# QI2lab/ray_trace_pb

Hardware: AMD Instinct MI355X
Metric: ray-surface intersections/sec at 1/2/4/8 MI355X; achieved HBM GB/s vs peak (higher is better)
Workload: dtype f64

## Files before the change

ray_trace_pb_amd/csrc/rtpb_core.hip:

```cpp
#include "rtpb_internal.h"

namespace rtpbi {

thread_local std::string g_last_error;

int fail(int code, const std::string& msg) {
    g_last_error = msg;
    return code;
}

PinnedStaging& pinned_staging() {
    thread_local PinnedStaging sg;
    return sg;
}

template <typename T>
void blob_layout(rtpb_plan& p) {
    p.off_mats = align256(p.surf.size() * sizeof(DevSurface<T>));
    p.off_table = p.off_mats + align256(p.mats.size() * sizeof(DevMaterial<T>));
    p.off_itab = p.off_table + align256(std::max<size_t>(p.table.size(), 2) * sizeof(T));
    p.blob_bytes = p.off_itab + align256(std::max<size_t>(p.itab.size(), 2) * sizeof(T));
}

DevMaterial<double> device_material(const rtpb_plan& p, size_t k) {
    const rtpb_material& m = p.mats[k];
    DevMaterial<double> d{};
    d.kind = m.kind;
    bool zero = m.kind == RTPB_SELLMEIER;
    for (int j = 0; j < 6; ++j) {
        d.c[j] = m.c[j];
        zero = zero && m.c[j] == 0.0;
    }
    if (zero) d.kind = VACUUM;
    d.table_off = p.table_off[k];
    d.table_len = m.kind == RTPB_TABLE ? m.table_len : 0;
    return d;
}

void build_indexed(rtpb_plan& p) {
    if (p.table.empty() || (p.feat & 2)) return;
    const size_t M = p.mats.size();
    int first = -1;
    for (size_t k = 0; k < M; ++k)
        if (p.mats[k].kind == RTPB_TABLE) { first = static_cast<int>(k); break; }
    if (first < 0) return;
    const int K = p.mats[first].table_len;
    const size_t S = p.surf.size();
    if (K <= 0 || static_cast<size_t>(K) * (M + 1 + S) > static_cast<size_t>(kLdsIndexedDoubles)) return;
    const double* keys0 = p.table.data() + 2 * static_cast<size_t>(p.table_off[first]);
    for (int j = 0; j < K; ++j) {
        const double kj = keys0[2 * j];
        if (kj != kj && j != K - 1) return;
        if (j > 0 && kj == kj && !(keys0[2 * (j - 1)] < kj)) return;
    }
    for (size_t k = 0; k < M; ++k) {
        if (p.mats[k].kind != RTPB_TABLE) continue;
        if (p.mats[k].table_len != K) return;
        const double* kk = p.table.data() + 2 * static_cast<size_t>(p.table_off[k]);
        for (int j = 0; j < K; ++j) {
            const double a = kk[2 * j], b = keys0[2 * j];
            if (a != a ? b == b : std::memcmp(&a, &b, sizeof(double)) != 0) return;
        }
    }
    std::vector<double> it(static_cast<size_t>(K) * (M + 1 + S));
    for (int j = 0; j < K; ++j) it[j] = keys0[2 * j];
    for (size_t k = 0; k < M; ++k) {
        const double* kk = p.table.data() + 2 * static_cast<size_t>(p.table_off[k]);
        const DevMaterial<double> d = device_material(p, k);
        for (int j = 0; j < K; ++j)
            it[K * (k + 1) + j] = p.mats[k].kind == RTPB_TABLE ? kk[2 * j + 1]
                                                               : material_n<double, false, false>(d, keys0[2 * j], static_cast<const double*>(nullptr));
    }
    for (size_t s = 0; s < S; ++s)
        for (int j = 0; j < K; ++j) it[K * (M + 1 + s) + j] = it[K * (s + 1) + j] / it[K * (s + 2) + j];
    p.itab.swap(it);
    p.nkeys = K;
    p.feat = (p.feat & ~(4 | 8)) | 16;
}

template <typename T>
std::vector<unsigned char> build_blob(const rtpb_plan& p) {
    const size_t S = p.surf.size(), M = p.mats.size(), off_mats = p.off_mats, off_table = p.off_table;
    std::vector<unsigned char> blob(p.blob_bytes, 0);
    auto* ds = reinterpret_cast<DevSurface<T>*>(blob.data());
    for (size_t k = 0; k < S; ++k) {
        DevSurface<double> d = lower_surface(p.surf[k]);
        lower_surface_media(d, device_material(p, k), device_material(p, k + 1));
        DevSurface<T>& o = ds[k];
        o.kind = d.kind;
        for (int j = 0; j < 3; ++j) {
            o.c[j] = T(d.c[j]);
            o.nrm[j] = T(d.nrm[j]);
            o.ax[j] = T(d.ax[j]);
        }
        o.R = T(d.R); o.R2 = T(d.R2); o.absR = T(d.absR); o.ap = T(d.ap); o.f = T(d.f); o.sin_a = T(d.sin_a);
        o.tol = T(d.tol); o.ap_sq = T(d.ap_sq); o.shell_lo = T(d.shell_lo); o.shell_hi = T(d.shell_hi);
        o.rR = T(d.rR); o.rf = T(d.rf); o.rcp_ok = d.rcp_ok;
        for (int j = 0; j < 3; ++j) o.nf[j] = T(d.nf[j]);
        o.nr = T(d.nr); o.rn2 = T(d.rn2);
        for (int j = 0; j < 3; ++j) {
            o.lF[j] = T(d.lF[j]);
            o.lB[j] = T(d.lB[j]);
        }
        o.ln1f = T(d.ln1f); o.lph = T(d.lph);
    }
    auto* dm = reinterpret_cast<DevMaterial<T>*>(blob.data() + off_mats);
    for (size_t k = 0; k < M; ++k) dm[k] = device_material(p, k);
    auto* tb = reinterpret_cast<T*>(blob.data() + off_table);
    for (size_t k = 0; k < p.table.size(); ++k) tb[k] = T(p.table[k]);
    auto* it = reinterpret_cast<T*>(blob.data() + p.off_itab);
    for (size_t k = 0; k < p.itab.size(); ++k) it[k] = T(p.itab[k]);
    return blob;
}

int plan_device_blob(rtpb_plan* p, int dev, void** out) {
    std::lock_guard<std::mutex> lk(p->mu);
    if (!p->blob[dev]) {
        std::vector<unsigned char> host = build_blob<double>(*p);
        DeviceGuard g(dev);
        void* d = nullptr;
        HIP_TRY(hipMalloc(&d, host.size()));
        hipError_t e = hipMemcpy(d, host.data(), host.size(), hipMemcpyHostToDevice);
        if (e != hipSuccess) {
            (void)hipFree(d);
            return fail(RTPB_E_HIP, std::string("hipMemcpy(plan): ") + hipGetErrorString(e));
        }
        p->blob[dev] = d;
    }
    *out = p->blob[dev];
    return RTPB_OK;
}

int check_device(int dev) {
    int n = 0;
    if (hipGetDeviceCount(&n) != hipSuccess || n <= 0) return fail(RTPB_E_NODEV, "no GPU device visible");
    if (dev < 0 || dev >= n || dev >= kMaxDevices)
        return fail(RTPB_E_NODEV, "device index " + std::to_string(dev) + " out of range");
    return RTPB_OK;
}

}

using namespace rtpbi;

extern "C" {

int rtpb_abi_version(void) { return RTPB_ABI_VERSION; }

const char* rtpb_last_error(void) { return g_last_error.c_str(); }

int rtpb_device_count(void) {
    int n = 0;
    if (hipGetDeviceCount(&n) != hipSuccess) return 0;
    return n;
}

int rtpb_plan_create(const rtpb_surface* surfaces, int32_t nsurf, const rtpb_material* materials, int32_t nmat,
                     int32_t dtype, rtpb_plan** plan_out) {
    if (!plan_out) return fail(RTPB_E_INVALID, "plan_out is NULL");
    *plan_out = nullptr;
    if (nsurf < 0 || (nsurf > 0 && !surfaces)) return fail(RTPB_E_INVALID, "bad surfaces array");
    if (nsurf > RTPB_MAX_SURFACES)
        return fail(RTPB_E_LIMIT, "more than RTPB_MAX_SURFACES (" + std::to_string(RTPB_MAX_SURFACES) + ") surfaces");
    if (nmat != nsurf + 1 || !materials)
        return fail(RTPB_E_INVALID, "length of materials should be len(surfaces) + 1");
    if (dtype != RTPB_F64 && dtype != RTPB_F32) return fail(RTPB_E_INVALID, "dtype must be RTPB_F64 or RTPB_F32");
    auto* p = new (std::nothrow) rtpb_plan();
    if (!p) return fail(RTPB_E_INVALID, "out of host memory");
    p->dtype = dtype;
    p->nsurf = nsurf;
    for (int k = 0; k < nsurf; ++k) {
        if (surfaces[k].kind < RTPB_FLAT || surfaces[k].kind > RTPB_PERFECT_LENS) {
            delete p;
            return fail(RTPB_E_INVALID, "surface " + std::to_string(k) + ": unknown kind");
        }
        p->surf.push_back(surfaces[k]);
        if (surfaces[k].kind == RTPB_PERFECT_LENS) p->feat |= 1;
    }
    for (int k = 0; k < nmat; ++k) {
        rtpb_material m = materials[k];
        if (m.kind < RTPB_CONSTANT || m.kind > RTPB_TABLE) {
            delete p;
            return fail(RTPB_E_INVALID, "material " + std::to_string(k) + ": unknown kind");
        }
        p->table_off.push_back(static_cast<int32_t>(p->table.size() / 2));
        if (m.kind == RTPB_POLY6) p->feat |= 3;
        if (m.kind == RTPB_TABLE) {
            if (m.table_len <= 0 || !m.table) {
                delete p;
                return fail(RTPB_E_INVALID, "material " + std::to_string(k) + ": empty table");
            }
            if (p->table.size() / 2 + m.table_len > RTPB_MAX_TABLE) {
                delete p;
                return fail(RTPB_E_LIMIT, "more than RTPB_MAX_TABLE wavelength table entries");
            }
            p->table.insert(p->table.end(), m.table, m.table + 2 * m.table_len);
            sort_table(p->table.data() + p->table.size() - 2 * m.table_len, m.table_len);
        }
        m.table = nullptr;
        p->mats.push_back(m);
    }
    if (!p->table.empty()) p->feat |= (p->table.size() / 2 <= static_cast<size_t>(kLdsTablePairs)) ? 4 : 8;
    if (g_indexed_materials.load()) build_indexed(*p);
    if (p->feat == 1) {
        bool lens_flat = true;
        for (const rtpb_surface& s : p->surf) {
            const DevSurface<double> d = lower_surface(s);
            lens_flat = lens_flat && (d.kind == FLAT || d.kind == PERFECT_LENS) &&
                        surface_geo(d.kind, d.rcp_ok) != kGeoGeneral;
        }
        if (lens_flat) p->feat |= 32;
    }
    blob_layout<double>(*p);
    *plan_out = p;
    return RTPB_OK;
}

int rtpb_plan_destroy(rtpb_plan* plan) {
    if (!plan) return RTPB_OK;
    for (int d = 0; d < kMaxDevices; ++d) {
        if (plan->blob[d]) {
            DeviceGuard g(d);
            (void)hipFree(plan->blob[d]);
        }
    }
    delete plan;
    return RTPB_OK;
}

}
```

ray_trace_pb_amd/csrc/rtpb_internal.h:

```cpp
#pragma once

#include <hip/hip_runtime.h>

#include <atomic>
#include <cmath>
#include <cstdio>
#include <cstring>
#include <mutex>
#include <string>
#include <thread>
#include <vector>

#include "rtpb.h"
#include "rtpb_math.h"

namespace rtpbi {

using namespace rtpb;

constexpr int kBlock = 256;
constexpr int kTraceBlock = 64;
constexpr int kMaxDevices = 64;

extern thread_local std::string g_last_error;
int fail(int code, const std::string& msg);

#define HIP_TRY(expr)                                                                          \
    do {                                                                                       \
        hipError_t e_ = (expr);                                                                \
        if (e_ != hipSuccess)                                                                  \
            return fail(RTPB_E_HIP, std::string(#expr ": ") + hipGetErrorString(e_));          \
    } while (0)

struct DeviceGuard {
    int prev = -1;
    explicit DeviceGuard(int dev) {
        if (hipGetDevice(&prev) != hipSuccess) prev = -1;
        if (prev != dev) (void)hipSetDevice(dev);
    }
    ~DeviceGuard() {
        int cur = -1;
        if (prev >= 0 && hipGetDevice(&cur) == hipSuccess && cur != prev) (void)hipSetDevice(prev);
    }
};

template <typename TIN, typename TS>
struct TraceArgs {
    const TIN* __restrict__ in;
    TS* __restrict__ out;
    const DevSurface<double>* __restrict__ surf;
    const DevMaterial<double>* __restrict__ mats;
    const double* __restrict__ table;
    const double* __restrict__ itab;
    int32_t* miss;
    int64_t n;
    int64_t in_fs;
    int64_t out_ps;
    int64_t out_fs;
    uint64_t mask_lo;
    uint64_t mask_hi;
    int32_t nsurf;
    int32_t ntable;
    int32_t nkeys;
};

constexpr int trace_feat_group(int feat) {
    return (feat == 0 || feat == 1 || feat == 4 || feat == 5 || feat == 33) ? 0 : 1;
}
template <typename TIN, typename TS, int GROUP>
hipError_t launch_trace_group(const TraceArgs<TIN, TS>& a, int il, int ol, int feat, hipStream_t st);
#define RTPB_TRACE_GROUP_EXTERN(TI, TS)                                                                             \
    extern template hipError_t launch_trace_group<TI, TS, 0>(const TraceArgs<TI, TS>&, int, int, int, hipStream_t); \
    extern template hipError_t launch_trace_group<TI, TS, 1>(const TraceArgs<TI, TS>&, int, int, int, hipStream_t);
RTPB_TRACE_GROUP_EXTERN(double, double)
RTPB_TRACE_GROUP_EXTERN(float, float)
RTPB_TRACE_GROUP_EXTERN(double, float)
RTPB_TRACE_GROUP_EXTERN(float, double)
#undef RTPB_TRACE_GROUP_EXTERN
template <typename TIN, typename TS>
inline hipError_t launch_trace(const TraceArgs<TIN, TS>& a, int il, int ol, int feat, hipStream_t st) {
    return trace_feat_group(feat) == 0 ? launch_trace_group<TIN, TS, 0>(a, il, ol, feat, st)
                                       : launch_trace_group<TIN, TS, 1>(a, il, ol, feat, st);
}
extern std::atomic<int> g_aos_staging, g_nt_stores, g_stage_input, g_host_chunk_mib, g_indexed_materials;
int set_buffer_pool_keep(int64_t k);
int set_buffer_dead_va_limit(int64_t bytes);

template <typename T> using cptr = const __attribute__((address_space(4))) T*;

template <typename T>
__device__ __forceinline__ DevSurface<T> load_surface(cptr<DevSurface<T>> p) {
    DevSurface<T> d;
    d.kind = p->kind;
    d.rcp_ok = p->rcp_ok;
    for (int j = 0; j < 3; ++j) {
        d.c[j] = p->c[j];
        d.nrm[j] = p->nrm[j];
        d.ax[j] = p->ax[j];
    }
    d.R = p->R; d.R2 = p->R2; d.absR = p->absR; d.ap = p->ap; d.f = p->f; d.sin_a = p->sin_a; d.tol = p->tol;
    d.ap_sq = p->ap_sq; d.shell_lo = p->shell_lo; d.shell_hi = p->shell_hi;
    d.rR = p->rR; d.rf = p->rf;
    d.nf[0] = p->nf[0]; d.nf[1] = p->nf[1]; d.nf[2] = p->nf[2];
    d.nr = p->nr; d.rn2 = p->rn2;
    for (int j = 0; j < 3; ++j) {
        d.lF[j] = p->lF[j];
        d.lB[j] = p->lB[j];
    }
    d.ln1f = p->ln1f; d.lph = p->lph;
    return d;
}

template <typename T>
__device__ __forceinline__ DevMaterial<T> load_material(cptr<DevMaterial<T>> p) {
    DevMaterial<T> d;
    d.kind = p->kind;
    d.table_off = p->table_off;
    d.table_len = p->table_len;
    d.pad = 0;
    for (int j = 0; j < 6; ++j) d.c[j] = p->c[j];
    return d;
}

template <typename TS, int LAYOUT>
__device__ __forceinline__ Ray<double> load_ray(const TS* __restrict__ in, int64_t i, int64_t fs) {
    Ray<double> r;
    if constexpr (LAYOUT == RTPB_AOS) {
        if constexpr (sizeof(TS) == 8) {
            const double2* p = reinterpret_cast<const double2*>(in + i * 8);
            const double2 a = p[0], b = p[1], c = p[2], d = p[3];
            r.x = a.x; r.y = a.y; r.z = b.x; r.dx = b.y; r.dy = c.x; r.dz = c.y; r.ph = d.x; r.wl = d.y;
        } else {
            const float4* p = reinterpret_cast<const float4*>(in + i * 8);
            const float4 a = p[0], b = p[1];
            r.x = a.x; r.y = a.y; r.z = a.z; r.dx = a.w; r.dy = b.x; r.dz = b.y; r.ph = b.z; r.wl = b.w;
        }
    } else {
        r.x = in[i]; r.y = in[fs + i]; r.z = in[2 * fs + i]; r.dx = in[3 * fs + i];
        r.dy = in[4 * fs + i]; r.dz = in[5 * fs + i]; r.ph = in[6 * fs + i]; r.wl = in[7 * fs + i];
#if defined(__HIP_DEVICE_COMPILE__)
        typedef double v2d __attribute__((ext_vector_type(2)));
        v2d a = {r.x, r.y}, b = {r.z, r.dx}, c = {r.dy, r.dz}, d = {r.ph, r.wl};
        asm volatile("" : "+v"(a), "+v"(b), "+v"(c), "+v"(d));
        r.x = a.x; r.y = a.y; r.z = b.x; r.dx = b.y; r.dy = c.x; r.dz = c.y; r.ph = d.x; r.wl = d.y;
#endif
    }
    return r;
}

template <typename TS, int LAYOUT>
__device__ __forceinline__ void store_ray(TS* __restrict__ out, int64_t i, int64_t fs, const Ray<double>& r) {
    if constexpr (LAYOUT == RTPB_AOS) {
        if constexpr (sizeof(TS) == 8) {
            double2* p = reinterpret_cast<double2*>(out + i * 8);
            p[0] = make_double2(r.x, r.y);
            p[1] = make_double2(r.z, r.dx);
            p[2] = make_double2(r.dy, r.dz);
            p[3] = make_double2(r.ph, r.wl);
        } else {
            float4* p = reinterpret_cast<float4*>(out + i * 8);
            p[0] = make_float4(float(r.x), float(r.y), float(r.z), float(r.dx));
            p[1] = make_float4(float(r.dy), float(r.dz), float(r.ph), float(r.wl));
        }
    } else {
        out[i] = TS(r.x); out[fs + i] = TS(r.y); out[2 * fs + i] = TS(r.z); out[3 * fs + i] = TS(r.dx);
        out[4 * fs + i] = TS(r.dy); out[5 * fs + i] = TS(r.dz); out[6 * fs + i] = TS(r.ph); out[7 * fs + i] = TS(r.wl);
    }
}

__device__ __forceinline__ bool plane_bit(uint64_t lo, uint64_t hi, int p) {
    return p < 64 ? ((lo >> p) & 1ull) : ((hi >> (p - 64)) & 1ull);
}

constexpr int kLdsTablePairs = 256;
constexpr int kLdsIndexedDoubles = 512;

__device__ __forceinline__ int key_index(const double* keys, int K, double wl) {
    if (wl != wl) return (K > 0 && keys[K - 1] != keys[K - 1]) ? K - 1 : -1;
    int lo = 0, hi = K;
    while (lo < hi) {
        const int mid = (lo + hi) >> 1;
        if (keys[mid] < wl) lo = mid + 1;
        else hi = mid;
    }
    return (lo < K && keys[lo] == wl) ? lo : -1;
}

constexpr int kTileBytes = 64 * 64;

typedef double v2d __attribute__((ext_vector_type(2)));
typedef float v4f __attribute__((ext_vector_type(4)));

template <typename TS>
__device__ __forceinline__ void tile_write(uint4* __restrict__ tile, int lane, const Ray<double>& r) {
    if constexpr (sizeof(TS) == 8) {
        const int sw = (lane >> 1) & 3;
        double2* t = reinterpret_cast<double2*>(tile);
        t[4 * lane + (0 ^ sw)] = make_double2(r.x, r.y);
        t[4 * lane + (1 ^ sw)] = make_double2(r.z, r.dx);
        t[4 * lane + (2 ^ sw)] = make_double2(r.dy, r.dz);
        t[4 * lane + (3 ^ sw)] = make_double2(r.ph, r.wl);
    } else {
        const int sw = (lane >> 2) & 1;
        float4* t = reinterpret_cast<float4*>(tile);
        t[2 * lane + (0 ^ sw)] = make_float4(float(r.x), float(r.y), float(r.z), float(r.dx));
        t[2 * lane + (1 ^ sw)] = make_float4(float(r.dy), float(r.dz), float(r.ph), float(r.wl));
    }
}

__device__ __forceinline__ uint64_t uniform_u64(uint64_t v) {
    return (static_cast<uint64_t>(__builtin_amdgcn_readfirstlane(static_cast<uint32_t>(v >> 32))) << 32) |
           static_cast<uint32_t>(__builtin_amdgcn_readfirstlane(static_cast<uint32_t>(v)));
}

template <typename TS, bool NT>
__device__ __forceinline__ void tile_flush(const uint4* __restrict__ tile, TS* __restrict__ plane, int64_t ray0,
                                           int64_t n, int lane) {
    constexpr int kRec = 8 * sizeof(TS);
    constexpr int kAux = NT ? (2 | 16) : 0;
    const int64_t left = n - ray0;
    const int nbytes = static_cast<int>((left < 64 ? left : 64) * kRec);
    const __amdgpu_buffer_rsrc_t rsrc = __builtin_amdgcn_make_buffer_rsrc(
        reinterpret_cast<void*>(uniform_u64(reinterpret_cast<uint64_t>(plane + ray0 * 8))), static_cast<short>(0),
        __builtin_amdgcn_readfirstlane(nbytes), 0x00020000);
    typedef unsigned int v4u __attribute__((ext_vector_type(4)));
    const v4u* t = reinterpret_cast<const v4u*>(tile);
    if constexpr (sizeof(TS) == 8) {
#pragma unroll
        for (int j = 0; j < 4; ++j) {
            const int c = lane + 64 * j, rr = c >> 2, pp = c & 3;
            __builtin_amdgcn_raw_buffer_store_b128(t[4 * rr + (pp ^ ((rr >> 1) & 3))], rsrc, c * 16, 0, kAux);
        }
    } else {
#pragma unroll
        for (int j = 0; j < 2; ++j) {
            const int c = lane + 64 * j, rr = c >> 1, pp = c & 1;
            __builtin_amdgcn_raw_buffer_store_b128(t[2 * rr + (pp ^ ((rr >> 2) & 1))], rsrc, c * 16, 0, kAux);
        }
    }
}

__device__ __forceinline__ void lds_wait() { asm volatile("s_waitcnt lgkmcnt(0)" ::: "memory"); }

__device__ __forceinline__ int xchg_ray(int lane) { return (lane & 1) ? 32 + (lane >> 1) : (lane >> 1); }

template <bool NT>
__device__ __forceinline__ void xchg_flush(float* __restrict__ plane, int64_t ray0, int64_t n, int lane,
                                           const Ray<double>& r) {
    constexpr int kAux = NT ? (2 | 16) : 0;
    typedef unsigned int v4u __attribute__((ext_vector_type(4)));
    const float lo[4] = {float(r.x), float(r.y), float(r.z), float(r.dx)};
    const float hi[4] = {float(r.dy), float(r.dz), float(r.ph), float(r.wl)};
    const bool odd = (lane & 1) != 0;
    v4u s0, s1;
#pragma unroll
    for (int k = 0; k < 4; ++k) {
        const int send = __float_as_int(odd ? lo[k] : hi[k]);
        const unsigned recv = static_cast<unsigned>(__builtin_amdgcn_mov_dpp(send, 0xB1, 0xF, 0xF, false));
        s0[k] = odd ? recv : __float_as_uint(lo[k]);
        s1[k] = odd ? __float_as_uint(hi[k]) : recv;
    }
    const int64_t left = n - ray0;
    const int nbytes = static_cast<int>((left < 64 ? left : 64) * 32);
    const __amdgpu_buffer_rsrc_t rsrc = __builtin_amdgcn_make_buffer_rsrc(
        reinterpret_cast<void*>(uniform_u64(reinterpret_cast<uint64_t>(plane + ray0 * 8))), static_cast<short>(0),
        __builtin_amdgcn_readfirstlane(nbytes), 0x00020000);
    __builtin_amdgcn_raw_buffer_store_b128(s0, rsrc, lane * 16, 0, kAux);
    __builtin_amdgcn_raw_buffer_store_b128(s1, rsrc, 1024 + lane * 16, 0, kAux);
}

template <typename TS>
__device__ __forceinline__ Ray<double> tile_load(uint4* __restrict__ tile, const TS* __restrict__ in, int64_t ray0,
                                                 int64_t n, int lane) {
    Ray<double> r;
    if constexpr (sizeof(TS) == 8) {
        double2* t = reinterpret_cast<double2*>(tile);
        const double2* g = reinterpret_cast<const double2*>(in + ray0 * 8);
        const int64_t nchunks = (n - ray0 < 64 ? n - ray0 : 64) * 4;
#pragma unroll
        for (int j = 0; j < 4; ++j) {
            const int c = lane + 64 * j, rr = c >> 2, pp = c & 3;
            const double2 v = g[c < nchunks ? c : nchunks - 4 + pp];
            t[4 * rr + (pp ^ ((rr >> 1) & 3))] = v;
        }
        lds_wait();
        const int sw = (lane >> 1) & 3;
        const double2 a = t[4 * lane + (0 ^ sw)], b = t[4 * lane + (1 ^ sw)], c = t[4 * lane + (2 ^ sw)],
                      d = t[4 * lane + (3 ^ sw)];
        r.x = a.x; r.y = a.y; r.z = b.x; r.dx = b.y; r.dy = c.x; r.dz = c.y; r.ph = d.x; r.wl = d.y;
    } else {
        float4* t = reinterpret_cast<float4*>(tile);
        const float4* g = reinterpret_cast<const float4*>(in + ray0 * 8);
        const int64_t nchunks = (n - ray0 < 64 ? n - ray0 : 64) * 2;
#pragma unroll
        for (int j = 0; j < 2; ++j) {
            const int c = lane + 64 * j, rr = c >> 1, pp = c & 1;
            const float4 v = g[c < nchunks ? c : nchunks - 2 + pp];
            t[2 * rr + (pp ^ ((rr >> 2) & 1))] = v;
        }
        lds_wait();
        const int sw = (lane >> 2) & 1;
        const float4 a = t[2 * lane + (0 ^ sw)], b = t[2 * lane + (1 ^ sw)];
        r.x = a.x; r.y = a.y; r.z = a.z; r.dx = a.w; r.dy = b.x; r.dz = b.y; r.ph = b.z; r.wl = b.w;
    }
    return r;
}

inline size_t align256(size_t x) { return (x + 255) & ~size_t(255); }

struct PinnedStaging {
    double* buf = nullptr;
    size_t cap = 0;
    hipEvent_t done = nullptr;

    int reserve(size_t bytes) {
        if (done) HIP_TRY(hipEventSynchronize(done));
        if (!done) HIP_TRY(hipEventCreateWithFlags(&done, hipEventDisableTiming));
        if (cap < bytes) {
            if (buf) HIP_TRY(hipHostFree(buf));
            buf = nullptr;
            cap = 0;
            HIP_TRY(hipHostMalloc(reinterpret_cast<void**>(&buf), bytes, hipHostMallocDefault));
            cap = bytes;
        }
        return RTPB_OK;
    }
    int upload(void* dev, size_t bytes, hipStream_t st) {
        HIP_TRY(hipMemcpyAsync(dev, buf, bytes, hipMemcpyHostToDevice, st));
        HIP_TRY(hipEventRecord(done, st));
        return RTPB_OK;
    }
};
PinnedStaging& pinned_staging();

}

struct rtpb_plan {
    int32_t dtype = RTPB_F64;
    int32_t nsurf = 0;
    std::vector<rtpb_surface> surf;
    std::vector<rtpb_material> mats;
    std::vector<int32_t> table_off;
    std::vector<double> table;
    int feat = 0;
    std::vector<double> itab;
    int32_t nkeys = 0;
    std::mutex mu;
    void* blob[rtpbi::kMaxDevices] = {};
    size_t off_mats = 0, off_table = 0, off_itab = 0, blob_bytes = 0;
};

namespace rtpbi {
int plan_device_blob(rtpb_plan* p, int dev, void** out);
DevMaterial<double> device_material(const rtpb_plan& p, size_t k);
int check_device(int dev);
}
```

ray_trace_pb_amd/csrc/rtpb_trace.hip:

```cpp

#include "rtpb_internal.h"

using namespace rtpbi;

namespace rtpbi {
std::atomic<int> g_aos_staging{1};
std::atomic<int> g_nt_stores{1};
std::atomic<int> g_stage_input{0};
std::atomic<int> g_host_chunk_mib{128};
std::atomic<int> g_indexed_materials{1};
}

namespace {

int popcount128(uint64_t lo, uint64_t hi) { return __builtin_popcountll(lo) + __builtin_popcountll(hi); }

struct TimingState {
    bool on = false;
    std::vector<std::pair<hipEvent_t, hipEvent_t>> pending;
    std::vector<std::pair<hipEvent_t, hipEvent_t>> pool;
};
thread_local TimingState g_timing;


int trace_impl(rtpb_plan* plan, int dev, const void* in, int in_dtype, int64_t n, int il, int64_t in_fs, void* out,
               int ol, int64_t out_ps, int64_t out_fs, uint64_t lo, uint64_t hi, hipStream_t st,
               int32_t* miss = nullptr) {
    void* blob = nullptr;
    int rc = plan_device_blob(plan, dev, &blob);
    if (rc) return rc;
    if (n == 0) return RTPB_OK;
    auto run = [&](auto tin, auto tag) -> hipError_t {
        using TIN = decltype(tin);
        using TS = decltype(tag);
        TraceArgs<TIN, TS> a{};
        a.in = static_cast<const TIN*>(in);
        a.out = static_cast<TS*>(out);
        a.surf = reinterpret_cast<const DevSurface<double>*>(blob);
        a.mats = reinterpret_cast<const DevMaterial<double>*>(static_cast<char*>(blob) + plan->off_mats);
        a.table = reinterpret_cast<const double*>(static_cast<char*>(blob) + plan->off_table);
        a.itab = reinterpret_cast<const double*>(static_cast<char*>(blob) + plan->off_itab);
        a.miss = miss;
        a.n = n;
        a.in_fs = in_fs;
        a.out_ps = out_ps;
        a.out_fs = out_fs;
        a.mask_lo = lo;
        a.mask_hi = hi;
        a.nsurf = plan->nsurf;
        a.ntable = static_cast<int32_t>(plan->table.size() / 2);
        a.nkeys = plan->nkeys;
        return launch_trace<TIN, TS>(a, il, ol, plan->feat, st);
    };
    hipEvent_t e0 = nullptr, e1 = nullptr;
    if (g_timing.on) {
        if (!g_timing.pool.empty()) {
            std::tie(e0, e1) = g_timing.pool.back();
            g_timing.pool.pop_back();
        } else {
            HIP_TRY(hipEventCreate(&e0));
            HIP_TRY(hipEventCreate(&e1));
        }
        HIP_TRY(hipEventRecord(e0, st));
    }
    hipError_t e;
    if (plan->dtype == RTPB_F64) e = in_dtype == RTPB_F64 ? run(double{}, double{}) : run(float{}, double{});
    else e = in_dtype == RTPB_F64 ? run(double{}, float{}) : run(float{}, float{});
    if (e != hipSuccess) return fail(RTPB_E_HIP, std::string("trace kernel launch: ") + hipGetErrorString(e));
    if (g_timing.on) {
        HIP_TRY(hipEventRecord(e1, st));
        g_timing.pending.emplace_back(e0, e1);
    }
    return RTPB_OK;
}

struct HostStage {
    std::mutex mu;
    hipStream_t st = nullptr;
    hipEvent_t ev[2] = {nullptr, nullptr};
    void* pin_in[2] = {nullptr, nullptr};
    void* pin_out[2] = {nullptr, nullptr};
    void* d_in[2] = {nullptr, nullptr};
    void* d_out[2] = {nullptr, nullptr};
    size_t in_bytes = 0, out_bytes = 0;
};
HostStage g_stage[kMaxDevices];

int stage_reserve(HostStage& hs, size_t in_bytes, size_t out_bytes) {
    if (!hs.st) {
        HIP_TRY(hipStreamCreateWithFlags(&hs.st, hipStreamNonBlocking));
        for (auto& e : hs.ev) HIP_TRY(hipEventCreateWithFlags(&e, hipEventDisableTiming));
    }
    if (in_bytes > hs.in_bytes || out_bytes > hs.out_bytes) {
        for (int k = 0; k < 2; ++k) {
            if (hs.pin_in[k]) (void)hipHostFree(hs.pin_in[k]);
            if (hs.pin_out[k]) (void)hipHostFree(hs.pin_out[k]);
            if (hs.d_in[k]) (void)hipFree(hs.d_in[k]);
            if (hs.d_out[k]) (void)hipFree(hs.d_out[k]);
            hs.pin_in[k] = hs.pin_out[k] = hs.d_in[k] = hs.d_out[k] = nullptr;
        }
        hs.in_bytes = hs.out_bytes = 0;
        for (int k = 0; k < 2; ++k) {
            HIP_TRY(hipHostMalloc(&hs.pin_in[k], in_bytes, hipHostMallocDefault));
            HIP_TRY(hipHostMalloc(&hs.pin_out[k], out_bytes, hipHostMallocDefault));
            HIP_TRY(hipMalloc(&hs.d_in[k], in_bytes));
            HIP_TRY(hipMalloc(&hs.d_out[k], out_bytes));
        }
        hs.in_bytes = in_bytes;
        hs.out_bytes = out_bytes;
    }
    return RTPB_OK;
}

void parallel_scatter(char* out, const char* staged, int nslots, int64_t slot_stride_bytes, int64_t piece_bytes,
                      int T) {
    const int64_t total = piece_bytes * nslots;
    T = static_cast<int>(std::max<int64_t>(1, std::min<int64_t>(T, total >> 23)));
    const int64_t per = (total + T - 1) / T;
    auto job = [&](int t) {
        int64_t lo = t * per, hi = std::min<int64_t>(total, lo + per);
        while (lo < hi) {
            const int64_t s = lo / piece_bytes, off = lo % piece_bytes;
            const int64_t len = std::min<int64_t>(hi - lo, piece_bytes - off);
            std::memcpy(out + s * slot_stride_bytes + off, staged + s * piece_bytes + off, static_cast<size_t>(len));
            lo += len;
        }
    };
    std::vector<std::thread> th;
    for (int t = 1; t < T; ++t) th.emplace_back(job, t);
    job(0);
    for (auto& x : th) x.join();
}

bool is_pinned_host(const void* p) {
    hipPointerAttribute_t attr;
    if (hipPointerGetAttributes(&attr, p) != hipSuccess) {
        (void)hipGetLastError();
        return false;
    }
    return attr.type == hipMemoryTypeHost;
}

int host_shard_pipeline(rtpb_plan* plan, int dev, const char* in, int in_dtype, char* out, int64_t n_rays, int64_t a,
                        int64_t b, size_t rec_in, size_t rec, int nslots, uint64_t lo, uint64_t hi, int T) {
    HostStage& hs = g_stage[dev];
    std::lock_guard<std::mutex> lk(hs.mu);
    DeviceGuard guard(dev);
#define HIP_TRY_SYNC(expr)                                                                     \
    do {                                                                                       \
        hipError_t e_ = (expr);                                                                \
        if (e_ != hipSuccess) {                                                                \
            (void)hipStreamSynchronize(hs.st);                                                 \
            return fail(RTPB_E_HIP, std::string(#expr ": ") + hipGetErrorString(e_));          \
        }                                                                                      \
    } while (0)
    const bool direct = is_pinned_host(out) && is_pinned_host(out + (int64_t(nslots) * n_rays * rec - 1));
    const int64_t target = int64_t(g_host_chunk_mib.load()) << 20;
    const int64_t chunk = std::min<int64_t>(b - a, std::max<int64_t>(1 << 16, target / int64_t(nslots * rec + rec_in)));
    int rc = stage_reserve(hs, chunk * rec_in, chunk * rec * nslots);
    if (rc) return rc;
    const int64_t nchunks = (b - a + chunk - 1) / chunk;
    auto scatter = [&](int64_t k) -> int {
        const int buf = static_cast<int>(k & 1);
        HIP_TRY(hipEventSynchronize(hs.ev[buf]));
        if (direct) return RTPB_OK;
        const int64_t c0 = a + k * chunk, m = std::min<int64_t>(chunk, b - c0);
        parallel_scatter(out + c0 * rec, static_cast<const char*>(hs.pin_out[buf]), nslots,
                         static_cast<int64_t>(n_rays * rec), static_cast<int64_t>(m * rec), T);
        return RTPB_OK;
    };
    for (int64_t k = 0; k < nchunks; ++k) {
        const int buf = static_cast<int>(k & 1);
        const int64_t c0 = a + k * chunk, m = std::min<int64_t>(chunk, b - c0);
        parallel_scatter(static_cast<char*>(hs.pin_in[buf]), in + c0 * rec_in, 1, 0, static_cast<int64_t>(m * rec_in), T);
        HIP_TRY_SYNC(hipMemcpyAsync(hs.d_in[buf], hs.pin_in[buf], m * rec_in, hipMemcpyHostToDevice, hs.st));
        rc = trace_impl(plan, dev, hs.d_in[buf], in_dtype, m, RTPB_AOS, 0, hs.d_out[buf], RTPB_AOS, m * 8, 0, lo, hi,
                        hs.st);
        if (rc) {
            (void)hipStreamSynchronize(hs.st);
            return rc;
        }
        if (direct)
            HIP_TRY_SYNC(hipMemcpy2DAsync(out + c0 * rec, n_rays * rec, hs.d_out[buf], m * rec, m * rec, nslots,
                                          hipMemcpyDeviceToHost, hs.st));
        else
            HIP_TRY_SYNC(hipMemcpyAsync(hs.pin_out[buf], hs.d_out[buf], m * rec * nslots, hipMemcpyDeviceToHost, hs.st));
        HIP_TRY_SYNC(hipEventRecord(hs.ev[buf], hs.st));
        if (k >= 1) {
            rc = scatter(k - 1);
            if (rc) {
                (void)hipStreamSynchronize(hs.st);
                return rc;
            }
        }
    }
    return scatter(nchunks - 1);
#undef HIP_TRY_SYNC
}

}

extern "C" {

int rtpb_shutdown(void) {
    rtpb_oneshot_clear();
    (void)rtpb_buffer_trim();
    for (int d = 0; d < kMaxDevices; ++d) {
        HostStage& hs = g_stage[d];
        std::lock_guard<std::mutex> lk(hs.mu);
        if (!hs.st) continue;
        DeviceGuard g(d);
        (void)hipStreamSynchronize(hs.st);
        for (int k = 0; k < 2; ++k) {
            if (hs.pin_in[k]) (void)hipHostFree(hs.pin_in[k]);
            if (hs.pin_out[k]) (void)hipHostFree(hs.pin_out[k]);
            if (hs.d_in[k]) (void)hipFree(hs.d_in[k]);
            if (hs.d_out[k]) (void)hipFree(hs.d_out[k]);
            hs.pin_in[k] = hs.pin_out[k] = hs.d_in[k] = hs.d_out[k] = nullptr;
            (void)hipEventDestroy(hs.ev[k]);
            hs.ev[k] = nullptr;
        }
        (void)hipStreamDestroy(hs.st);
        hs.st = nullptr;
        hs.in_bytes = hs.out_bytes = 0;
    }
    return RTPB_OK;
}

int rtpb_trace(const rtpb_plan* plan_c, int32_t device, const void* rays_in, int32_t in_dtype, int64_t n_rays,
               int32_t in_layout, int64_t in_field_stride, void* out, int32_t out_layout, int64_t out_plane_stride,
               int64_t out_field_stride, uint64_t plane_mask_lo, uint64_t plane_mask_hi, void* stream) {
    return rtpb_trace_checked(plan_c, device, rays_in, in_dtype, n_rays, in_layout, in_field_stride, out, out_layout,
                              out_plane_stride, out_field_stride, plane_mask_lo, plane_mask_hi, stream, nullptr);
}

static_assert(sizeof(rtpb_trace_call) == 5 * 8 + 6 * 8 + 4 * 4, "rtpb_trace_call: no padding (bindings mirror it)");

int rtpb_trace_packed(const rtpb_trace_call* c) {
    if (!c) return fail(RTPB_E_INVALID, "call is NULL");
    return rtpb_trace_checked(c->plan, c->device, c->rays_in, c->in_dtype, c->n_rays, c->in_layout, c->in_field_stride,
                              c->out, c->out_layout, c->out_plane_stride, c->out_field_stride, c->plane_mask_lo,
                              c->plane_mask_hi, c->stream, c->table_miss);
}

int rtpb_trace_checked(const rtpb_plan* plan_c, int32_t device, const void* rays_in, int32_t in_dtype,
                       int64_t n_rays, int32_t in_layout, int64_t in_field_stride, void* out, int32_t out_layout,
                       int64_t out_plane_stride, int64_t out_field_stride, uint64_t plane_mask_lo,
                       uint64_t plane_mask_hi, void* stream, int32_t* table_miss) {
    auto* plan = const_cast<rtpb_plan*>(plan_c);
    if (!plan) return fail(RTPB_E_INVALID, "plan is NULL");
    int rc = check_device(device);
    if (rc) return rc;
    if (n_rays < 0) return fail(RTPB_E_INVALID, "n_rays < 0");
    const int nplanes = 2 * plan->nsurf + 1;
    if (nplanes < 128 && ((nplanes >= 64 ? (plane_mask_hi >> (nplanes - 64)) : (plane_mask_hi | (plane_mask_lo >> nplanes))) != 0))
        return fail(RTPB_E_INVALID, "plane mask selects planes beyond 2*nsurf");
    const int nslots = popcount128(plane_mask_lo, plane_mask_hi);
    if (in_layout != RTPB_AOS && in_layout != RTPB_SOA) return fail(RTPB_E_INVALID, "bad in_layout");
    if (out_layout != RTPB_AOS && out_layout != RTPB_SOA) return fail(RTPB_E_INVALID, "bad out_layout");
    if (in_dtype != RTPB_F64 && in_dtype != RTPB_F32) return fail(RTPB_E_INVALID, "bad in_dtype");
    if (in_dtype != plan->dtype && in_layout != RTPB_AOS)
        return fail(RTPB_E_INVALID, "SOA input must have the plan's storage type");
    if (n_rays > 0 && !rays_in) return fail(RTPB_E_INVALID, "rays_in is NULL");
    if (n_rays > 0 && nslots > 0 && !out) return fail(RTPB_E_INVALID, "out is NULL");
    const size_t w = plan->dtype == RTPB_F64 ? 8 : 4;
    if (in_layout == RTPB_AOS && (reinterpret_cast<uintptr_t>(rays_in) % 16))
        return fail(RTPB_E_INVALID, "AOS rays_in must be 16-byte aligned");
    if (out_layout == RTPB_AOS && nslots > 0 &&
        ((reinterpret_cast<uintptr_t>(out) % 16) || ((out_plane_stride * w) % 16)))
        return fail(RTPB_E_INVALID, "AOS out and its plane stride must be 16-byte aligned");
    if (nslots > 1 && out_plane_stride < 8 * n_rays) return fail(RTPB_E_INVALID, "out_plane_stride < 8*n_rays");
    if (in_layout == RTPB_SOA && in_field_stride < n_rays) return fail(RTPB_E_INVALID, "in_field_stride < n_rays");
    if (out_layout == RTPB_SOA && out_field_stride < n_rays) return fail(RTPB_E_INVALID, "out_field_stride < n_rays");
    DeviceGuard g(device);
    return trace_impl(plan, device, rays_in, in_dtype, n_rays, in_layout, in_field_stride, out, out_layout,
                      out_plane_stride, out_field_stride, plane_mask_lo, plane_mask_hi, static_cast<hipStream_t>(stream),
                      table_miss);
}

int rtpb_trace_host(const rtpb_plan* plan_c, const void* rays_in, int32_t in_dtype, int64_t n_rays, void* out,
                    uint64_t plane_mask_lo, uint64_t plane_mask_hi, const int32_t* devices, int32_t n_devices) {
    auto* plan = const_cast<rtpb_plan*>(plan_c);
    if (!plan) return fail(RTPB_E_INVALID, "plan is NULL");
    if (n_rays < 0) return fail(RTPB_E_INVALID, "n_rays < 0");
    if (in_dtype != RTPB_F64 && in_dtype != RTPB_F32) return fail(RTPB_E_INVALID, "bad in_dtype");
    std::vector<int> devs;
    if (!devices || n_devices <= 0) devs.push_back(0);
    else devs.assign(devices, devices + n_devices);
    for (int d : devs) {
        int rc = check_device(d);
        if (rc) return rc;
    }
    const int nslots = popcount128(plane_mask_lo, plane_mask_hi);
    if (n_rays == 0 || nslots == 0) return RTPB_OK;
    if (!rays_in || !out) return fail(RTPB_E_INVALID, "NULL host buffer");
    const size_t rec = 8 * (plan->dtype == RTPB_F64 ? 8 : 4);
    const size_t rec_in = 8 * (in_dtype == RTPB_F64 ? 8 : 4);
    const int G = static_cast<int>(devs.size());
    const unsigned hw = std::max(2u, std::thread::hardware_concurrency());
    const int copy_threads = static_cast<int>(std::max(2u, std::min(16u, hw / static_cast<unsigned>(G))));
    std::vector<int> rcs(G, RTPB_OK);
    std::vector<std::string> errs(G);
    auto worker = [&](int g) {
        const int dev = devs[g];
        const int64_t a = n_rays * g / G, b = n_rays * (g + 1) / G;
        if (b <= a) return;
        rcs[g] = host_shard_pipeline(plan, dev, static_cast<const char*>(rays_in), in_dtype, static_cast<char*>(out),
                                     n_rays, a, b, rec_in, rec, nslots, plane_mask_lo, plane_mask_hi, copy_threads);
        if (rcs[g]) errs[g] = g_last_error;
    };
    if (G == 1) {
        worker(0);
    } else {
        std::vector<std::thread> th;
        for (int g = 0; g < G; ++g) th.emplace_back(worker, g);
        for (auto& t : th) t.join();
    }
    for (int g = 0; g < G; ++g)
        if (rcs[g]) return fail(rcs[g], "device " + std::to_string(devs[g]) + ": " + errs[g]);
    return RTPB_OK;
}

int rtpb_set_tuning(const char* key, int64_t value) {
    if (!key) return fail(RTPB_E_INVALID, "key is NULL");
    if (std::strcmp(key, "aos_staging") == 0) {
        if (value < 0 || value > 2) return fail(RTPB_E_INVALID, "aos_staging must be 0, 1 or 2");
        g_aos_staging.store(static_cast<int>(value));
        return RTPB_OK;
    }
    if (std::strcmp(key, "nt_stores") == 0) {
        g_nt_stores.store(value != 0);
        return RTPB_OK;
    }
    if (std::strcmp(key, "stage_input") == 0) {
        g_stage_input.store(value != 0);
        return RTPB_OK;
    }
    if (std::strcmp(key, "host_chunk_mib") == 0) {
        if (value < 1 || value > 4096) return fail(RTPB_E_INVALID, "host_chunk_mib must be in [1, 4096]");
        g_host_chunk_mib.store(static_cast<int>(value));
        return RTPB_OK;
    }
    if (std::strcmp(key, "indexed_materials") == 0) {
        g_indexed_materials.store(value != 0);
        return RTPB_OK;
    }
    if (std::strcmp(key, "buffer_pool_buffers") == 0) return set_buffer_pool_keep(value);
    if (std::strcmp(key, "buffer_dead_va_limit") == 0) return set_buffer_dead_va_limit(value);
    return fail(RTPB_E_INVALID, std::string("unknown tuning key ") + key);
}

int rtpb_timing_enable(int32_t on) {
    g_timing.on = on != 0;
    return RTPB_OK;
}

int rtpb_timing_collect(double* total_ms, int64_t* launches) {
    double tot = 0.0;
    int64_t cnt = 0;
    for (auto& pr : g_timing.pending) {
        HIP_TRY(hipEventSynchronize(pr.second));
        float ms = 0.f;
        HIP_TRY(hipEventElapsedTime(&ms, pr.first, pr.second));
        tot += ms;
        ++cnt;
        g_timing.pool.push_back(pr);
    }
    g_timing.pending.clear();
    if (total_ms) *total_ms = tot;
    if (launches) *launches = cnt;
    return RTPB_OK;
}

}
```

ray_trace_pb_amd/csrc/rtpb_trace_kernel.h:

```cpp

#pragma once

#include "rtpb_internal.h"

namespace rtpbi {


constexpr int trace_block(int out_layout, int store) {
    return (out_layout == RTPB_AOS && (store & 1)) ? kTraceBlock : 256;
}

template <typename TIN, typename TS, int IN_LAYOUT, int OUT_LAYOUT, int STORE, int WPE, int FEAT>
__global__ __launch_bounds__(trace_block(OUT_LAYOUT, STORE)) __attribute__((amdgpu_waves_per_eu(WPE, 8)))
void trace_kernel(TraceArgs<TIN, TS> a) {
    constexpr int kB = trace_block(OUT_LAYOUT, STORE);
    using T = double;
    constexpr bool kStaged = (STORE & 1) && OUT_LAYOUT == RTPB_AOS;
    constexpr bool kNT = (STORE & 2) != 0;
    constexpr bool kXchg = (STORE & 16) != 0;
    static_assert(!kXchg || (kStaged && sizeof(TS) == 4 && kB == 64), "exchange flush: staged float32 AOS");
    constexpr bool kFinal = (STORE & 8) != 0;
    constexpr bool kLens = (FEAT & 1) != 0, kPoly = (FEAT & 2) != 0;
    constexpr int kKinds = (FEAT & 32) != 0 ? kKindsLensFlat : kKindsAll;
    constexpr bool kTabLds = (FEAT & 12) == 4, kTabGlobal = (FEAT & 8) != 0, kIdx = (FEAT & 16) != 0;
    extern __shared__ double lds_table[];
    if constexpr (kTabLds || kIdx) {
        const int cnt = kIdx ? a.nkeys * (2 * a.nsurf + 2) : 2 * a.ntable;
        const double* src = kIdx ? a.itab : a.table;
        for (int k = threadIdx.x; k < cnt; k += kB) lds_table[k] = src[k];
        if constexpr (kB > 64) __syncthreads();
    }
    __shared__ uint4 tiles[kB / 64][kFinal ? 1 : 2][kTileBytes / 16 * sizeof(TS) / 8];
    const int lane = threadIdx.x & 63;
    auto body = [&](const int64_t blk) {
    const int64_t i = kXchg ? blk * kB + xchg_ray(lane) : blk * kB + threadIdx.x;
    const int64_t ray0 = kXchg ? blk * kB
                               : static_cast<int64_t>(uniform_u64(static_cast<uint64_t>(i - lane)));
    if (ray0 >= a.n) return;
    const bool valid = i < a.n;
    uint4* tile_a = tiles[threadIdx.x >> 6][0];
    uint4* tile_b = tiles[threadIdx.x >> 6][kFinal ? 0 : 1];
    Ray<T> r;
    if constexpr (kStaged && IN_LAYOUT == RTPB_AOS && (STORE & 4) && std::is_same<TIN, TS>::value)
        r = tile_load<TS>(tile_b, a.in, ray0, a.n, lane);
    else r = load_ray<TIN, IN_LAYOUT>(a.in, valid ? i : a.n - 1, a.in_fs);
    const T wl0 = r.wl;
    const Rcp<T> iwl = make_wl_rcp(wl0);
    TS* __restrict__ out = a.out;
    const cptr<DevSurface<T>> surf = (cptr<DevSurface<T>>)(a.surf);
    const cptr<DevMaterial<T>> mats = (cptr<DevMaterial<T>>)(a.mats);
    const cptr<T> table = (cptr<T>)(a.table);
    const int widx = kIdx ? key_index(lds_table, a.nkeys, wl0) : -1;
    if constexpr (kIdx || kTabLds || kTabGlobal) {
        if (a.miss != nullptr) {
            bool miss = false;
            if constexpr (kIdx) {
                miss = widx < 0;
            } else {
                for (int k = 0; k <= a.nsurf; ++k) {
                    const DevMaterial<T> m = load_material<T>(mats + k);
                    if (m.kind == TABLE)
                        miss = miss || !(kTabLds ? table_has_key(m, wl0, static_cast<const double*>(lds_table))
                                                 : table_has_key(m, wl0, table));
                }
            }
            if (valid && miss) a.miss[0] = 1;
        }
    }
    const bool all_idx = kIdx && __builtin_amdgcn_ballot_w64(widx < 0) == 0;
    const T w2 = wl0 * wl0;
    const bool vac_one = __builtin_amdgcn_ballot_w64(!(w2 != T(0) && w2 - w2 == T(0))) == 0;
    auto surface = [&](int s) -> DevSurface<T> {
        DevSurface<T> d = load_surface<T>(surf + s);
        if ((d.rcp_ok & 16) && vac_one) d.rcp_ok |= 4 | ((d.rcp_ok & 32) ? 8 : 0);
        if ((d.rcp_ok & kLensUniVac) && vac_one) d.rcp_ok |= kLensUni;
        if constexpr (kIdx) {
            if (all_idx && !(d.rcp_ok & 4)) {
                d.nr = lds_table[a.nkeys * (a.nsurf + 2 + s) + widx];
                d.rcp_ok |= 4;
            }
        }
        return d;
    };
    auto mat_n = [&](cptr<DevMaterial<T>> mp) -> T {
        if constexpr (kIdx) {
            if (widx >= 0) return lds_table[a.nkeys * (1 + static_cast<int>(mp - mats)) + widx];
            return material_n<T, false, false>(load_material<T>(mp), wl0, table);
        } else if constexpr (kTabLds) {
            return material_n<T, kPoly, true>(load_material<T>(mp), wl0, lds_table);
        } else {
            return material_n<T, kPoly, kTabGlobal>(load_material<T>(mp), wl0, table);
        }
    };
    if constexpr (kFinal) {
        T n_cur = mat_n(mats);
        for (int s = 0; s < a.nsurf; s += 2) {
            const T n_mid = mat_n(mats + s + 1);
            Ray<T> mid;
            propagate_surface_emit<T, kLens, kNoAt, kKinds>(surface(s), r, n_cur, n_mid, iwl, [](const Ray<T>&) {}, mid);
            if (s + 1 < a.nsurf) {
                const T n_next = mat_n(mats + s + 2);
                propagate_surface_emit<T, kLens, kNoAt, kKinds>(surface(s + 1), mid, n_mid, n_next, iwl, [](const Ray<T>&) {},
                                                        r);
                n_cur = n_next;
            } else {
                r = mid;
                n_cur = n_mid;
            }
        }
        if constexpr (kXchg) {
            xchg_flush<kNT>(out, ray0, a.n, lane, r);
        } else if constexpr (kStaged) {
            tile_write<TS>(tile_b, lane, r);
            lds_wait();
            tile_flush<TS, kNT>(tile_b, out, ray0, a.n, lane);
        } else if (valid) {
            store_ray<TS, OUT_LAYOUT>(out, i, a.out_fs, r);
        }
        return;
    }
    int64_t slot_off = 0;
    if (a.mask_lo & 1ull) {
        if constexpr (kXchg) {
            xchg_flush<kNT>(out, ray0, a.n, lane, r);
        } else if constexpr (kStaged) {
            tile_write<TS>(tile_a, lane, r);
            lds_wait();
            tile_flush<TS, kNT>(tile_a, out, ray0, a.n, lane);
        } else if (valid) {
            store_ray<TS, OUT_LAYOUT>(out, i, a.out_fs, r);
        }
        slot_off += a.out_ps;
    }
    auto one = [&](int s, const Ray<T>& in, T n_in, Ray<T>& res, T& n_res) {
        const T n_next = mat_n(mats + s + 1);
        const int p = 2 * s + 1;
        const bool st_at = plane_bit(a.mask_lo, a.mask_hi, p);
        const bool st_after = plane_bit(a.mask_lo, a.mask_hi, p + 1);
        const int64_t off_at = slot_off;
        slot_off += st_at ? a.out_ps : 0;
        const int64_t off_after = slot_off;
        slot_off += st_after ? a.out_ps : 0;
        auto emit_at = [&](const Ray<T>& at) {
            if constexpr (kXchg) {
                if (st_at) xchg_flush<kNT>(out + off_at, ray0, a.n, lane, at);
            } else if constexpr (kStaged) {
                if (st_at) tile_write<TS>(tile_a, lane, at);
            } else {
                if (valid && st_at) store_ray<TS, OUT_LAYOUT>(out + off_at, i, a.out_fs, at);
            }
        };
        propagate_surface_emit<T, kLens, 0, kKinds>(surface(s), in, n_in, n_next, iwl, emit_at, res);
        if constexpr (kXchg) {
            if (st_after) xchg_flush<kNT>(out + off_after, ray0, a.n, lane, res);
        } else if constexpr (kStaged) {
            if (st_after) tile_write<TS>(tile_b, lane, res);
            if (st_at || st_after) lds_wait();
            if (st_at) tile_flush<TS, kNT>(tile_a, out + off_at, ray0, a.n, lane);
            if (st_after) tile_flush<TS, kNT>(tile_b, out + off_after, ray0, a.n, lane);
        } else if (valid) {
            if (st_after) store_ray<TS, OUT_LAYOUT>(out + off_after, i, a.out_fs, res);
        }
        n_res = n_next;
    };
    T n_cur = mat_n(mats);
    for (int s = 0; s < a.nsurf; s += 2) {
        Ray<T> mid;
        T n_mid;
        one(s, r, n_cur, mid, n_mid);
        if (s + 1 < a.nsurf) {
            one(s + 1, mid, n_mid, r, n_cur);
        } else {
            r = mid;
            n_cur = n_mid;
        }
    }
    };
    body(static_cast<int64_t>(blockIdx.x));
}



template <typename TI, typename T, int IL, int OL, int ST, int W, int FEAT>
hipError_t launch_w(const TraceArgs<TI, T>& a, hipStream_t st) {
    constexpr int kB = trace_block(OL, ST);
    const int64_t blocks = (a.n + kB - 1) / kB;
    const size_t lds = (FEAT & 16)        ? static_cast<size_t>(a.nkeys) * (2 * a.nsurf + 2) * sizeof(double)
                       : (FEAT & 12) == 4 ? static_cast<size_t>(a.ntable) * 2 * sizeof(double) : 0;
    hipLaunchKernelGGL((trace_kernel<TI, T, IL, OL, ST, W, FEAT>), dim3(static_cast<unsigned>(blocks)), dim3(kB), lds,
                       st, a);
    return hipGetLastError();
}

template <typename TI, typename T, int IL, int OL, int ST, int GROUP>
hipError_t launch_one(const TraceArgs<TI, T>& a, int feat, hipStream_t st) {
#define RTPB_WPE(F) (((ST & 8) && sizeof(T) == 8 && (F) != 15) ? 6 : 1)
    if constexpr (GROUP == 0) {
        switch (feat) {
        case 0: return launch_w<TI, T, IL, OL, ST, RTPB_WPE(0), 0>(a, st);
        case 1: return launch_w<TI, T, IL, OL, ST, RTPB_WPE(1), 1>(a, st);
        case 4: return launch_w<TI, T, IL, OL, ST, RTPB_WPE(4), 4>(a, st);
        case 5: return launch_w<TI, T, IL, OL, ST, RTPB_WPE(5), 5>(a, st);
        case 33: return launch_w<TI, T, IL, OL, ST, RTPB_WPE(33), 33>(a, st);
        default: return hipErrorInvalidValue;
        }
    } else {
        switch (feat) {
        case 16: return launch_w<TI, T, IL, OL, ST, RTPB_WPE(16), 16>(a, st);
        case 17: return launch_w<TI, T, IL, OL, ST, RTPB_WPE(17), 17>(a, st);
        default: return launch_w<TI, T, IL, OL, ST, RTPB_WPE(15), 15>(a, st);
        }
    }
#undef RTPB_WPE
}

template <typename TI, typename T, int G>
hipError_t launch_trace_group(const TraceArgs<TI, T>& a, int il, int ol, int feat, hipStream_t st) {
    const int staging = g_aos_staging.load();
    const bool staged = staging != 0;
    const bool nt = g_nt_stores.load() != 0;
    constexpr bool kF32 = sizeof(T) == 4;
    const bool xchg = kF32 && staging == 2 && nt;
    const int last = 2 * a.nsurf;
    const bool final_only = a.nsurf > 0 && (last < 64 ? (a.mask_lo == (1ull << last) && a.mask_hi == 0)
                                                      : (a.mask_lo == 0 && a.mask_hi == (1ull << (last - 64))));
    if (final_only && ol == RTPB_AOS && il == RTPB_AOS && staged && nt && !g_stage_input.load())
    {
        if constexpr (kF32) {
            if (xchg) return launch_one<TI, T, RTPB_AOS, RTPB_AOS, 27, G>(a, feat, st);
        }
        return launch_one<TI, T, RTPB_AOS, RTPB_AOS, 11, G>(a, feat, st);
    }
    if constexpr (!std::is_same<TI, T>::value) {
        if (ol == RTPB_SOA) return launch_one<TI, T, RTPB_AOS, RTPB_SOA, 0, G>(a, feat, st);
        if (!staged) return launch_one<TI, T, RTPB_AOS, RTPB_AOS, 0, G>(a, feat, st);
        if constexpr (kF32) {
            if (xchg) return launch_one<TI, T, RTPB_AOS, RTPB_AOS, 19, G>(a, feat, st);
        }
        return nt ? launch_one<TI, T, RTPB_AOS, RTPB_AOS, 3, G>(a, feat, st) : launch_one<TI, T, RTPB_AOS, RTPB_AOS, 1, G>(a, feat, st);
    }
    if (ol == RTPB_AOS) {
        if (!staged)
            return il == RTPB_AOS ? launch_one<TI, T, RTPB_AOS, RTPB_AOS, 0, G>(a, feat, st) : launch_one<TI, T, RTPB_SOA, RTPB_AOS, 0, G>(a, feat, st);
        if (nt && il == RTPB_AOS && g_stage_input.load()) return launch_one<TI, T, RTPB_AOS, RTPB_AOS, 7, G>(a, feat, st);
        if constexpr (kF32) {
            if (xchg && il == RTPB_AOS) return launch_one<TI, T, RTPB_AOS, RTPB_AOS, 19, G>(a, feat, st);
        }
        if (nt)
            return il == RTPB_AOS ? launch_one<TI, T, RTPB_AOS, RTPB_AOS, 3, G>(a, feat, st) : launch_one<TI, T, RTPB_SOA, RTPB_AOS, 3, G>(a, feat, st);
        return il == RTPB_AOS ? launch_one<TI, T, RTPB_AOS, RTPB_AOS, 1, G>(a, feat, st) : launch_one<TI, T, RTPB_SOA, RTPB_AOS, 1, G>(a, feat, st);
    }
    if (il == RTPB_AOS) return launch_one<TI, T, RTPB_AOS, RTPB_SOA, 0, G>(a, feat, st);
    return launch_one<TI, T, RTPB_SOA, RTPB_SOA, 0, G>(a, feat, st);
}


}
```

Baseline: 82.41 billion.

## Add monochromatic fast path using precomputed per-surface index ratios and flags

When the indexed material table has a single wavelength key, the host precomputes per-surface reciprocal indices, rcp/lens flags, and wavelength reciprocals into the itab tail. The kernel checks via a wave ballot whether every ray's wavelength matches that key. If so, it takes a specialized path that reads indices straight from constant memory, skips the LDS table staging, the key binary search, and the per-surface flag fixups, and uses the uniform-media propagation variant. This adds a second kernel instantiation, which raises code size and register pressure, plus a ballot check on every wave.

```diff
diff --git a/ray_trace_pb_amd/csrc/rtpb_core.hip b/ray_trace_pb_amd/csrc/rtpb_core.hip
--- a/ray_trace_pb_amd/csrc/rtpb_core.hip
+++ b/ray_trace_pb_amd/csrc/rtpb_core.hip
@@ -73,6 +73,23 @@
     }
     for (size_t s = 0; s < S; ++s)
         for (int j = 0; j < K; ++j) it[K * (M + 1 + s) + j] = it[K * (s + 1) + j] / it[K * (s + 2) + j];
+    if (K == 1 && std::fabs(it[0]) >= 0x1p-120 && std::fabs(it[0]) < 0x1p120) {
+        const double key = it[0];
+        const size_t t0 = it.size();
+        it.resize(t0 + 2 * S + kMonoTail);
+        for (size_t s = 0; s < S; ++s) {
+            const double n2 = it[s + 2];
+            it[t0 + s] = 1.0 / n2;
+            DevSurface<double> d = lower_surface(p.surf[s]);
+            lower_surface_media(d, device_material(p, s), device_material(p, s + 1));
+            const int64_t bits = (d.rcp_ok & ~(4 | 8)) | 4 | (host_rcp_ok(n2) ? 8 : 0) |
+                                 ((d.rcp_ok & kLensUniVac) ? kLensUni : 0);
+            std::memcpy(&it[t0 + S + s], &bits, sizeof(double));
+        }
+        it[t0 + 2 * S] = 1.0 / key;
+        it[t0 + 2 * S + 1] = Const<double>::two_pi / key;
+        p.mono = true;
+    }
     p.itab.swap(it);
     p.nkeys = K;
     p.feat = (p.feat & ~(4 | 8)) | 16;
diff --git a/ray_trace_pb_amd/csrc/rtpb_internal.h b/ray_trace_pb_amd/csrc/rtpb_internal.h
--- a/ray_trace_pb_amd/csrc/rtpb_internal.h
+++ b/ray_trace_pb_amd/csrc/rtpb_internal.h
@@ -62,6 +62,7 @@
     int32_t nsurf;
     int32_t ntable;
     int32_t nkeys;
+    int32_t mono;
 };
 
 constexpr int trace_feat_group(int feat) {
@@ -82,7 +83,8 @@
     return trace_feat_group(feat) == 0 ? launch_trace_group<TIN, TS, 0>(a, il, ol, feat, st)
                                        : launch_trace_group<TIN, TS, 1>(a, il, ol, feat, st);
 }
-extern std::atomic<int> g_aos_staging, g_nt_stores, g_stage_input, g_host_chunk_mib, g_indexed_materials;
+extern std::atomic<int> g_aos_staging, g_nt_stores, g_stage_input, g_host_chunk_mib, g_indexed_materials,
+    g_mono_plans;
 int set_buffer_pool_keep(int64_t k);
 int set_buffer_dead_va_limit(int64_t bytes);
 
@@ -174,6 +176,7 @@
 
 constexpr int kLdsTablePairs = 256;
 constexpr int kLdsIndexedDoubles = 512;
+constexpr int kMonoTail = 2;
 
 __device__ __forceinline__ int key_index(const double* keys, int K, double wl) {
     if (wl != wl) return (K > 0 && keys[K - 1] != keys[K - 1]) ? K - 1 : -1;
@@ -345,6 +348,7 @@
     int feat = 0;
     std::vector<double> itab;
     int32_t nkeys = 0;
+    bool mono = false;
     std::mutex mu;
     void* blob[rtpbi::kMaxDevices] = {};
     size_t off_mats = 0, off_table = 0, off_itab = 0, blob_bytes = 0;
diff --git a/ray_trace_pb_amd/csrc/rtpb_trace.hip b/ray_trace_pb_amd/csrc/rtpb_trace.hip
--- a/ray_trace_pb_amd/csrc/rtpb_trace.hip
+++ b/ray_trace_pb_amd/csrc/rtpb_trace.hip
@@ -9,6 +9,7 @@
 std::atomic<int> g_stage_input{0};
 std::atomic<int> g_host_chunk_mib{128};
 std::atomic<int> g_indexed_materials{1};
+std::atomic<int> g_mono_plans{1};
 }
 
 namespace {
@@ -50,6 +51,7 @@
         a.nsurf = plan->nsurf;
         a.ntable = static_cast<int32_t>(plan->table.size() / 2);
         a.nkeys = plan->nkeys;
+        a.mono = (plan->mono && g_mono_plans.load()) ? 1 : 0;
         return launch_trace<TIN, TS>(a, il, ol, plan->feat, st);
     };
     hipEvent_t e0 = nullptr, e1 = nullptr;
@@ -345,6 +347,10 @@
         g_indexed_materials.store(value != 0);
         return RTPB_OK;
     }
+    if (std::strcmp(key, "mono_plans") == 0) {
+        g_mono_plans.store(value != 0);
+        return RTPB_OK;
+    }
     if (std::strcmp(key, "buffer_pool_buffers") == 0) return set_buffer_pool_keep(value);
     if (std::strcmp(key, "buffer_dead_va_limit") == 0) return set_buffer_dead_va_limit(value);
     return fail(RTPB_E_INVALID, std::string("unknown tuning key ") + key);
diff --git a/ray_trace_pb_amd/csrc/rtpb_trace_kernel.h b/ray_trace_pb_amd/csrc/rtpb_trace_kernel.h
--- a/ray_trace_pb_amd/csrc/rtpb_trace_kernel.h
+++ b/ray_trace_pb_amd/csrc/rtpb_trace_kernel.h
@@ -24,10 +24,14 @@
     constexpr int kKinds = (FEAT & 32) != 0 ? kKindsLensFlat : kKindsAll;
     constexpr bool kTabLds = (FEAT & 12) == 4, kTabGlobal = (FEAT & 8) != 0, kIdx = (FEAT & 16) != 0;
     extern __shared__ double lds_table[];
-    if constexpr (kTabLds || kIdx) {
+    auto stage_table = [&]() {
         const int cnt = kIdx ? a.nkeys * (2 * a.nsurf + 2) : 2 * a.ntable;
         const double* src = kIdx ? a.itab : a.table;
         for (int k = threadIdx.x; k < cnt; k += kB) lds_table[k] = src[k];
+    };
+    constexpr bool kLateTable = kIdx && kB == 64;
+    if constexpr ((kTabLds || kIdx) && !kLateTable) {
+        stage_table();
         if constexpr (kB > 64) __syncthreads();
     }
     __shared__ uint4 tiles[kB / 64][kFinal ? 1 : 2][kTileBytes / 16 * sizeof(TS) / 8];
@@ -44,14 +48,21 @@
     if constexpr (kStaged && IN_LAYOUT == RTPB_AOS && (STORE & 4) && std::is_same<TIN, TS>::value)
         r = tile_load<TS>(tile_b, a.in, ray0, a.n, lane);
     else r = load_ray<TIN, IN_LAYOUT>(a.in, valid ? i : a.n - 1, a.in_fs);
-    const T wl0 = r.wl;
-    const Rcp<T> iwl = make_wl_rcp(wl0);
     TS* __restrict__ out = a.out;
     const cptr<DevSurface<T>> surf = (cptr<DevSurface<T>>)(a.surf);
     const cptr<DevMaterial<T>> mats = (cptr<DevMaterial<T>>)(a.mats);
     const cptr<T> table = (cptr<T>)(a.table);
-    const int widx = kIdx ? key_index(lds_table, a.nkeys, wl0) : -1;
-    if constexpr (kIdx || kTabLds || kTabGlobal) {
+    const cptr<T> itab = (cptr<T>)(a.itab);
+    auto trace = [&](auto mono_tag, Ray<T> r) {
+    constexpr bool kMono = decltype(mono_tag)::value;
+    constexpr int kMedia = kMono ? kUniMedia : 0;
+    const int mono_tail = 2 * a.nsurf + 2;
+    if constexpr (kLateTable && !kMono) stage_table();
+    const T wl0 = kMono ? itab[0] : r.wl;
+    const Rcp<T> iwl = kMono ? Rcp<T>{wl0, itab[mono_tail + 2 * a.nsurf], true, itab[mono_tail + 2 * a.nsurf + 1]}
+                             : make_wl_rcp(wl0);
+    const int widx = (kIdx && !kMono) ? key_index(lds_table, a.nkeys, wl0) : -1;
+    if constexpr ((kIdx || kTabLds || kTabGlobal) && !kMono) {
         if (a.miss != nullptr) {
             bool miss = false;
             if constexpr (kIdx) {
@@ -67,11 +78,20 @@
             if (valid && miss) a.miss[0] = 1;
         }
     }
-    const bool all_idx = kIdx && __builtin_amdgcn_ballot_w64(widx < 0) == 0;
-    const T w2 = wl0 * wl0;
-    const bool vac_one = __builtin_amdgcn_ballot_w64(!(w2 != T(0) && w2 - w2 == T(0))) == 0;
+    const bool all_idx = kIdx && !kMono && __builtin_amdgcn_ballot_w64(widx < 0) == 0;
+    bool vac_one = true;
+    if constexpr (!kMono) {
+        const T w2 = wl0 * wl0;
+        vac_one = __builtin_amdgcn_ballot_w64(!(w2 != T(0) && w2 - w2 == T(0))) == 0;
+    }
     auto surface = [&](int s) -> DevSurface<T> {
         DevSurface<T> d = load_surface<T>(surf + s);
+        if constexpr (kMono) {
+            d.nr = itab[a.nsurf + 2 + s];
+            d.rn2 = itab[mono_tail + s];
+            d.rcp_ok = reinterpret_cast<cptr<int32_t>>(itab + mono_tail + a.nsurf + s)[0];
+            return d;
+        }
         if ((d.rcp_ok & 16) && vac_one) d.rcp_ok |= 4 | ((d.rcp_ok & 32) ? 8 : 0);
         if ((d.rcp_ok & kLensUniVac) && vac_one) d.rcp_ok |= kLensUni;
         if constexpr (kIdx) {
@@ -83,7 +103,9 @@
         return d;
     };
     auto mat_n = [&](cptr<DevMaterial<T>> mp) -> T {
-        if constexpr (kIdx) {
+        if constexpr (kMono) {
+            return itab[1 + static_cast<int>(mp - mats)];
+        } else if constexpr (kIdx) {
             if (widx >= 0) return lds_table[a.nkeys * (1 + static_cast<int>(mp - mats)) + widx];
             return material_n<T, false, false>(load_material<T>(mp), wl0, table);
         } else if constexpr (kTabLds) {
@@ -97,10 +119,10 @@
         for (int s = 0; s < a.nsurf; s += 2) {
             const T n_mid = mat_n(mats + s + 1);
             Ray<T> mid;
-            propagate_surface_emit<T, kLens, kNoAt, kKinds>(surface(s), r, n_cur, n_mid, iwl, [](const Ray<T>&) {}, mid);
+            propagate_surface_emit<T, kLens, kNoAt | kMedia, kKinds>(surface(s), r, n_cur, n_mid, iwl, [](const Ray<T>&) {}, mid);
             if (s + 1 < a.nsurf) {
                 const T n_next = mat_n(mats + s + 2);
-                propagate_surface_emit<T, kLens, kNoAt, kKinds>(surface(s + 1), mid, n_mid, n_next, iwl, [](const Ray<T>&) {},
+                propagate_surface_emit<T, kLens, kNoAt | kMedia, kKinds>(surface(s + 1), mid, n_mid, n_next, iwl, [](const Ray<T>&) {},
                                                         r);
                 n_cur = n_next;
             } else {
@@ -150,7 +172,7 @@
                 if (valid && st_at) store_ray<TS, OUT_LAYOUT>(out + off_at, i, a.out_fs, at);
             }
         };
-        propagate_surface_emit<T, kLens, 0, kKinds>(surface(s), in, n_in, n_next, iwl, emit_at, res);
+        propagate_surface_emit<T, kLens, kMedia, kKinds>(surface(s), in, n_in, n_next, iwl, emit_at, res);
         if constexpr (kXchg) {
             if (st_after) xchg_flush<kNT>(out + off_after, ray0, a.n, lane, res);
         } else if constexpr (kStaged) {
@@ -175,6 +197,15 @@
             n_cur = n_mid;
         }
     }
+    };
+    if constexpr (kIdx) {
+        if (a.mono && __builtin_amdgcn_ballot_w64(__builtin_bit_cast(uint64_t, r.wl) !=
+                                                  reinterpret_cast<cptr<uint64_t>>(itab)[0]) == 0) {
+            trace(std::true_type(), r);
+            return;
+        }
+    }
+    trace(std::false_type(), r);
     };
     body(static_cast<int64_t>(blockIdx.x));
 }
```

After: 81.90 billion. Within noise of the previous version (-0.6%).
